# skyepurchase/MeatModeler

Hardware: AMD Instinct MI355X
Metric: descriptor-match pairs/sec + BA residuals/sec, 500×1080p frames, 1/2/4/8 GPU (higher is better)
Workload: dtype u8/int32 (match), f64 (BA); 1 GPU; 500 frames 1920x1080, 4000 ORB kpts/frame, BF Hamming 2-NN + ratio, track linking, 2-view DLT, full BA (TRF, Schur, f64 MFMA Cholesky); frames=500, height=1080, width=1920, nfeatures=4000, parallelism=pairs/points x1

## Files before the change

meatmodeler_amd/csrc/mm_common.h:

```cpp
#pragma once
#include <hip/hip_runtime.h>
#include <cstdarg>
#include <cstdio>
#include <cstring>
#include <vector>
#include "../../include/meatmodeler.h"

struct mm_prof_rec {
    const char *name;
    hipEvent_t a, b;
};

struct mm_ctx {
    int device;
    hipStream_t stream;
    char err[512];
    int prof = 0;
    char prof_only[64] = {0};
    std::vector<mm_prof_rec> recs;
    std::vector<hipEvent_t> pool;
    hipStream_t aux = nullptr;
    hipEvent_t ev_fork = nullptr, ev_join = nullptr;
    bool attr_chol_fused = false, attr_chol_bwd = false, attr_chol_batch = false;
    int cu_count = 0, fused_wgs = 0, chol_last_path = -1, debug_abandon = 0;
    bool chol_avoid_fused = false;
    bool chol_strict_budget = false;
    hipEvent_t fused_ev = nullptr;
    bool fused_ev_pending = false;
    bool fused_no_event = false;
    int link_last_variant = -1;
    void *cam_tab = nullptr;
    int cam_tab_cap = 0, cam_tab_F = 0;
    const double *cam_tab_for = nullptr;
    bool cam_tab_hold = false;
    const double *fx_cams = nullptr;
    int fx_F = 0;
    bool fx_tab_ok = false;
    void *host_board = nullptr;
    unsigned long long host_board_seq = 0;
    void *batch_dev = nullptr, *batch_host = nullptr;
    size_t batch_dev_cap = 0, batch_host_cap = 0;
    bool jvp_rows_deferred = false;
    const double *jvp_partial = nullptr;
    unsigned jvp_n_wg = 0;
    const void *chol_init_done = nullptr;
    int chol_init_sides = 0;
    int batch_last = -1;
};
// ... 54 lines not shown
    bool fused;
    int sides;
    unsigned grid_fused, grid_bwd;
};
struct mm_chol_init_args {
    int32_t *info, *flags;
    size_t nflags;
    unsigned long long *sentinel_buf;
    size_t nsent;
    unsigned long long *lpub;
    size_t nlpub;
    unsigned long long *Linv;
    size_t nblk;
};
bool mm_chol_init_plan(mm_ctx *ctx, int n, int half_bandwidth, int32_t *info, void *ws, size_t ws_bytes, mm_chol_init_args *out, int *sides, int *bwb);
void mm_chol_init_done(mm_ctx *ctx, const void *ws, int sides);
struct mm_damp_spec {
    const double *B, *C, *si;
    const double *gh2, *d11;
    double Delta, min_damping;
    double *damp_out;
    const double *reg;
};
int mm_ba_schur_solve_damped(mm_ctx *ctx, const mm_ba_problem *pb, const double *cams, const double *pts, const mm_damp_spec *dmp,
                             double *Bd, double *Cd, const double *gc, const double *gp, double *S, double *v, double *Cinv,
                             int half_bandwidth, int32_t *info, void *ws_schur, size_t ws_schur_bytes, void *ws_chol,
                             size_t ws_chol_bytes);
int mm_chol_solve_gated(mm_ctx *ctx, double *A, int n, double *b, int nrhs, int half_bandwidth, int32_t *info, void *ws,
                        size_t ws_bytes, const int32_t *slab_ready, int cams_per_slab, int n_cams, int sym_mode);

struct mm_batch_prob {
    mm_ba_problem pb;
    int64_t n, nc;
    double *x, *x_new, *g, *si, *gh, *ghs, *gn, *q1, *w, *q2, *s1, *s2;
    double *B, *Bd, *C, *Cd, *Cinv, *u1, *Jq2, *dp, *v, *S;
    double *r0, *r1, *r2, *r3, *d11, *bs, *damp, *board;
    int32_t *info;
    void *ctab_x, *ctab_new;
    double *res_partial;
    unsigned *md_counter;
    double *md_partial;
    double *jvp_partial;
    double *backsub_T;
    double *schur_partial, *schur_camtab;
    int32_t *schur_seg_done, *schur_desc;
    mm_chol_layout chol;
    int32_t half_bw, chol_sym_mirror;
    uint32_t g_vec, g_res, g_jvp, g_pblk, g_obs, g_pts, g_scale, g_damp, g_prep, g_pairs, g_chol, g_bwd, g_coef, g_zero;
    void *mailbox;
};
// ... 86 lines not shown
```

meatmodeler_amd/csrc/mm_ctx.hip:

```cpp
#include "mm_common.h"

extern "C" {

int mm_abi_version(void) { return 3; }

int mm_ctx_create(int device, void *hip_stream, mm_ctx **out) {
    if (!out) return MM_ERR_ARG;
    int n = 0;
    if (hipGetDeviceCount(&n) != hipSuccess || device < 0 || device >= n) return MM_ERR_HIP;
    mm_ctx *c = new mm_ctx();
    c->device = device;
    c->stream = (hipStream_t)hip_stream;
    c->err[0] = 0;
    if (hipSetDevice(device) != hipSuccess) {
        delete c;
        return MM_ERR_HIP;
    }
    if (hipDeviceGetAttribute(&c->cu_count, hipDeviceAttributeMultiprocessorCount, device) != hipSuccess) c->cu_count = 0;
    *out = c;
    return MM_OK;
}

void mm_ctx_destroy(mm_ctx *ctx) {
    if (!ctx) return;
// ... 68 lines not shown
const char *mm_last_error(mm_ctx *ctx) { return ctx ? ctx->err : "null context"; }

int mm_ctx_sync(mm_ctx *ctx) {
    if (!ctx) return MM_ERR_ARG;
    MM_HIP(ctx, hipStreamSynchronize(ctx->stream));
    mm_chol_release_budget(ctx);
    return MM_OK;
}

long long mm_ctx_control(mm_ctx *ctx, int what, long long value) {
    if (!ctx) return MM_ERR_ARG;
    switch (what) {
        case MM_CTL_CHOL_FORCE_ABANDON: ctx->debug_abandon = value < 0 ? 0 : (int)value; return MM_OK;
        case MM_CTL_CHOL_LAST_PATH: return ctx->chol_last_path;
        case MM_CTL_CHOL_RESERVED: return ctx->fused_wgs;
        case MM_CTL_CU_COUNT: return ctx->cu_count;
        case MM_CTL_CHOL_AVOID_FUSED: {
            const long long prev = ctx->chol_avoid_fused ? 1 : 0;
            if (value >= 0) ctx->chol_avoid_fused = value != 0;
            return prev;
        }
        case MM_CTL_LINK_LAST_VARIANT: return ctx->link_last_variant;
        case MM_CTL_BATCH_LAST: return ctx->batch_last;
        default: return mm_fail(ctx, MM_ERR_ARG, "mm_ctx_control: unknown request %d", what);
    }
}

struct mm_timer {
    hipEvent_t a, b;
};

int mm_timer_create(mm_ctx *ctx, void **timer_out) {
    if (!ctx || !timer_out) return MM_ERR_ARG;
    mm_timer *t = new mm_timer();
    MM_HIP(ctx, hipEventCreate(&t->a));
    MM_HIP(ctx, hipEventCreate(&t->b));
    *timer_out = t;
    return MM_OK;
}
int mm_timer_start(mm_ctx *ctx, void *timer) {
    if (!ctx || !timer) return MM_ERR_ARG;
    MM_HIP(ctx, hipEventRecord(((mm_timer *)timer)->a, ctx->stream));
    return MM_OK;
}
int mm_timer_stop(mm_ctx *ctx, void *timer) {
    if (!ctx || !timer) return MM_ERR_ARG;
// ... 21 lines not shown
```

meatmodeler_amd/csrc/schur.hip:

```cpp
#include "ba_eval.h"
#include "chol_init.h"

namespace {

constexpr int SR_WIN = 256;

__global__ __launch_bounds__(256) void point_inverse_kernel(int P, const double *__restrict__ Cd,
                                                            double *__restrict__ Cinv) {
    int p = blockIdx.x * 256 + threadIdx.x;
    if (p >= P) return;
    const double *c = Cd + (size_t)p * 6;
    const double a = c[0], b = c[1], d = c[2], e = c[3], f = c[4], g = c[5];
    const double m00 = e * g - f * f, m01 = d * f - b * g, m02 = b * f - d * e;
    const double det = a * m00 + b * m01 + d * m02;
    const double id = 1.0 / det;
    double *o = Cinv + (size_t)p * 6;
    o[0] = m00 * id;
    o[1] = m01 * id;
    o[2] = m02 * id;
    o[3] = (a * g - d * d) * id;
    o[4] = (b * d - a * f) * id;
    o[5] = (a * e - b * b) * id;
}

// ... 311 lines not shown
            const int sl = i / slabs.cams_per_slab;
            if (atomicAdd(slabs.done + sl, 1) == slabs.seg_count[sl] - 1)
                __hip_atomic_store(slabs.ready + sl, 1, __ATOMIC_RELEASE, __HIP_MEMORY_SCOPE_AGENT);
        }
    }
}


struct CamPQ {
    double P[9], q[3];
};
__device__ __forceinline__ double fast_rcp(double x) {
    double y = __builtin_amdgcn_rcp(x);
    double e = fma(-x, y, 1.0);
    y = fma(y, e, y);
    e = fma(-x, y, 1.0);
    return fma(y, e, y);
}

struct LeanJ {
    double Jc[2][6];
    double Jp[2][3];
};
__device__ __forceinline__ void lean_eval(const CamPQ &c, const double *__restrict__ Ks, const double *__restrict__ Jr,
                                          double X0, double X1, double X2, LeanJ &o) {
    const double u0 = fma(c.P[0], X0, fma(c.P[1], X1, fma(c.P[2], X2, c.q[0])));
    const double u1 = fma(c.P[3], X0, fma(c.P[4], X1, fma(c.P[5], X2, c.q[1])));
    const double u2 = fma(c.P[6], X0, fma(c.P[7], X1, fma(c.P[8], X2, c.q[2])));
    const double iz = fast_rcp(u2);
    const double p[2] = {u0 * iz, u1 * iz};
#pragma unroll
    for (int m = 0; m < 2; ++m) {
#pragma unroll
        for (int k = 0; k < 3; ++k) {
            o.Jp[m][k] = fma(-p[m], c.P[6 + k], c.P[3 * m + k]) * iz;
            o.Jc[m][3 + k] = fma(-p[m], Ks[6 + k], Ks[3 * m + k]) * iz;
        }
        const double g0 = X1 * o.Jp[m][2] - X2 * o.Jp[m][1];
        const double g1 = X2 * o.Jp[m][0] - X0 * o.Jp[m][2];
        const double g2 = X0 * o.Jp[m][1] - X1 * o.Jp[m][0];
#pragma unroll
        for (int k = 0; k < 3; ++k) o.Jc[m][k] = fma(g0, Jr[k], fma(g1, Jr[3 + k], g2 * Jr[6 + k]));
    }
}

constexpr int SLAB2 = 32;
struct ChunkDesc {
    int32_t i, f2, e_begin, e_end, sidx, c_first, n_ch, pad;
};
template <bool FORCE>
__device__ __forceinline__ CamPQ cam_pq_scalar(const double *__restrict__ t) {
    CamPQ v;
#pragma unroll
    for (int k = 0; k < 9; ++k) v.P[k] = FORCE ? uniform_f64(t[k]) : t[k];
#pragma unroll
    for (int k = 0; k < 3; ++k) v.q[k] = FORCE ? uniform_f64(t[9 + k]) : t[9 + k];
    return v;
}
template <bool FORCE_UNIFORM>
__device__ __forceinline__ void schur_pairs_body(const mm_ba_problem pb, const double *__restrict__ camtab,
                                                                    const ChunkDesc *__restrict__ desc,
                                                                    const double *__restrict__ pts,
                                                                    const double *__restrict__ Cinv,
                                                                    const double *__restrict__ gp,
                                                                    double *partial, const double *__restrict__ Bd,
                                                                    const double *__restrict__ gc, double *S, double *v,
// ... 43 lines not shown
#pragma unroll
    for (int q = 0; q < 42; ++q) acc[q] = 0.0;
    auto load_xc = [&](int p, double (&x)[12]) {
        if (p >= 0) {
            const double *Xp = pts + (size_t)p * 3, *ci = Cinv + (size_t)p * 6;
            x[0] = Xp[0];
            x[1] = Xp[1];
            x[2] = Xp[2];
#pragma unroll
            for (int q = 0; q < 6; ++q) x[3 + q] = ci[q];
            if (d == 0) {
                x[9] = gp[(size_t)p * 3];
                x[10] = gp[(size_t)p * 3 + 1];
                x[11] = gp[(size_t)p * 3 + 2];
            }
        }
    };
    auto pair_body = [&](int p, bool self, const double (&x)[12]) {
        const double X0 = x[0], X1 = x[1], X2 = x[2];
        const double q00 = x[3], q01 = x[4], q02 = x[5], q11 = x[6], q12 = x[7], q22 = x[8];
        LeanJ a;
        lean_eval(cp_i, Ks, Jr_i, X0, X1, X2, a);
        double Z[2][3];
#pragma unroll
        for (int m = 0; m < 2; ++m) {
            Z[m][0] = a.Jp[m][0] * q00 + a.Jp[m][1] * q01 + a.Jp[m][2] * q02;
            Z[m][1] = a.Jp[m][0] * q01 + a.Jp[m][1] * q11 + a.Jp[m][2] * q12;
            Z[m][2] = a.Jp[m][0] * q02 + a.Jp[m][1] * q12 + a.Jp[m][2] * q22;
        }
        double M[2][2], T[2][6];
        if (d == 0) {
            if (self) {
                const double g0 = x[9], g1 = x[10], g2 = x[11];
                const double z0 = Z[0][0] * g0 + Z[0][1] * g1 + Z[0][2] * g2, z1 = Z[1][0] * g0 + Z[1][1] * g1 + Z[1][2] * g2;
#pragma unroll
                for (int q = 0; q < 6; ++q) acc[36 + q] += a.Jc[0][q] * z0 + a.Jc[1][q] * z1;
            }
#pragma unroll
            for (int m = 0; m < 2; ++m)
#pragma unroll
                for (int n_ = 0; n_ < 2; ++n_) M[m][n_] = Z[m][0] * a.Jp[n_][0] + Z[m][1] * a.Jp[n_][1] + Z[m][2] * a.Jp[n_][2];
#pragma unroll
            for (int b = 0; b < 6; ++b) {
                T[0][b] = M[0][0] * a.Jc[0][b] + M[0][1] * a.Jc[1][b];
                T[1][b] = M[1][0] * a.Jc[0][b] + M[1][1] * a.Jc[1][b];
            }
        } else {
            LeanJ b2;
            lean_eval(cp_2, Ks, Jr_2, X0, X1, X2, b2);
#pragma unroll
            for (int m = 0; m < 2; ++m)
#pragma unroll
                for (int n_ = 0; n_ < 2; ++n_) M[m][n_] = Z[m][0] * b2.Jp[n_][0] + Z[m][1] * b2.Jp[n_][1] + Z[m][2] * b2.Jp[n_][2];
#pragma unroll
            for (int b = 0; b < 6; ++b) {
                T[0][b] = M[0][0] * b2.Jc[0][b] + M[0][1] * b2.Jc[1][b];
                T[1][b] = M[1][0] * b2.Jc[0][b] + M[1][1] * b2.Jc[1][b];
            }
        }
#pragma unroll
        for (int q = 0; q < 6; ++q)
#pragma unroll
            for (int b = 0; b < 6; ++b) acc[q * 6 + b] += a.Jc[0][q] * T[0][b] + a.Jc[1][q] * T[1][b];
    };
    double xc[12];
    load_xc(p_next, xc);
    int p_cur = p_next;
    bool self_cur = self_next;
    {
        const int en = e + 64;
        p_next = en < e_end ? point_of(en) : -1;
        self_next = en < e_end && self_of(en);
    }
#pragma clang loop unroll(disable)
    for (; e - lane < e_end; e += 64) {
        double xn[12];
        load_xc(p_next, xn);
        const int p_nn_e = e + 128;
        const int p_nn = p_nn_e < e_end ? point_of(p_nn_e) : -1;
        const bool self_nn = p_nn_e < e_end && self_of(p_nn_e);
        if (p_cur >= 0) pair_body(p_cur, self_cur, xc);
#pragma unroll
        for (int q = 0; q < 12; ++q) xc[q] = xn[q];
        p_cur = p_next;
        self_cur = self_next;
        p_next = p_nn;
// ... 68 lines not shown
                                                                    const double *__restrict__ gp,
                                                                    double *partial, const double *__restrict__ Bd,
                                                                    const double *__restrict__ gc, double *S, double *v,
                                                                    int32_t *seg_done, SlabSync slabs, unsigned wg_begin,
                                                                    unsigned wg_total) {
    schur_pairs_body<false>(pb, camtab, desc, pts, Cinv, gp, partial, Bd, gc, S, v, seg_done, slabs, wg_begin, wg_total, blockIdx.x);
}
__global__ __launch_bounds__(256) void zero_batch_kernel(const mm_batch_prob *__restrict__ tab, const int32_t *__restrict__ list) {
    const mm_batch_prob &bp = tab[list[blockIdx.y]];
    if (blockIdx.x >= bp.g_zero) return;
    double2 *S2 = reinterpret_cast<double2 *>(bp.S);
    const int64_t n2 = bp.nc * bp.nc / 2;
    for (int64_t i = (int64_t)blockIdx.x * 256 + threadIdx.x; i < n2; i += (int64_t)bp.g_zero * 256) S2[i] = make_double2(0.0, 0.0);
}
__global__ __launch_bounds__(64 * SP_WAVES, 2) void schur_pairs_batch_kernel(const mm_batch_prob *__restrict__ tab, const int32_t *__restrict__ list) {
    const mm_batch_prob &bp = tab[list[blockIdx.y]];
    if (blockIdx.x >= bp.g_pairs) return;
    SlabSync none = {};
    schur_pairs_body<true>(bp.pb, bp.schur_camtab, (const ChunkDesc *)bp.schur_desc, bp.x + bp.nc, bp.Cinv, bp.g + bp.nc, bp.schur_partial, bp.Bd,
                     bp.g, bp.S, bp.v, bp.schur_seg_done, none, 0u, bp.g_pairs, blockIdx.x);
}




__global__ void slab_flag_kernel(int32_t *flags, int s) {
    __hip_atomic_store(flags + s, 1, __ATOMIC_RELEASE, __HIP_MEMORY_SCOPE_AGENT);
}

__global__ void schur_diag_fill_kernel(mm_ba_problem pb, const double *__restrict__ Bd, const double *__restrict__ gc,
                                       double *__restrict__ S, double *__restrict__ v) {
    const int i = blockIdx.x;
    if (pb.cam_ptr[i + 1] != pb.cam_ptr[i]) return;
    const size_t n = (size_t)pb.F * 6;
    if (threadIdx.x < 36) S[((size_t)i * 6 + threadIdx.x / 6) * n + (size_t)i * 6 + threadIdx.x % 6] = Bd[(size_t)i * 36 + threadIdx.x];
    if (threadIdx.x < 6) v[(size_t)i * 6 + threadIdx.x] = gc[(size_t)i * 6 + threadIdx.x];
}

struct PrepExtra {
    mm_damp_spec dmp;
    int zero_bwb;
    int chol_init;
    mm_chol_init_args init;
};
__device__ __forceinline__ void schur_prepare_body(mm_ba_problem pb, const double *__restrict__ cams,
                                                            double *__restrict__ Bd, const double *__restrict__ Cd,
// ... 167 lines not shown
    if (pb->O == 0) return MM_OK;
    MM_LAUNCH(ctx, "pairs_count_kernel", pairs_count_kernel, dim3((unsigned)((pb->O + 255) / 256)), dim3(256), 0, *pb, cnt,
              span_out);
    return MM_OK;
}

extern "C" int mm_ba_pairs_emit(mm_ctx *ctx, const mm_ba_problem *pb, const int64_t *offsets, int span, int32_t *key,
                                int32_t *pair_o, int32_t *pair_o2) {
    if (!ctx) return MM_ERR_ARG;
    if (!pb || !offsets || !key || !pair_o || !pair_o2 || span < 0) return mm_fail(ctx, MM_ERR_ARG, "mm_ba_pairs_emit: bad argument");
    if (pb->O == 0) return MM_OK;
    if ((int64_t)pb->F * (span + 1) > 0x7fffffffLL) return mm_fail(ctx, MM_ERR_ARG, "mm_ba_pairs_emit: F * (span + 1) overflows the key");
    MM_LAUNCH(ctx, "pairs_emit_kernel", pairs_emit_kernel, dim3((unsigned)((pb->O + 255) / 256)), dim3(256), 0, *pb, offsets,
              span, key, pair_o, pair_o2);
    return MM_OK;
}

extern "C" size_t mm_ba_schur_workspace_bytes(const mm_ba_problem *pb) {
    if (!pb || pb->n_chunks <= 0) return 0;
    return mm_align_up((size_t)pb->n_chunks * 42 * sizeof(double), 256)  +
           mm_align_up((size_t)pb->n_seg * sizeof(int32_t), 256)  +
           mm_align_up(2 * MAX_SLABS * sizeof(int32_t), 256)  +
           mm_align_up((size_t)pb->F * CAMTAB2 * sizeof(double), 256)  +
           mm_align_up((size_t)pb->n_chunks * 32, 256) ;
}

namespace {
bool schur_pairs_lean() {
    static const bool lean = [] {
        const char *e = getenv("MM_SCHUR_PAIRS");
        return !(e && e[0] == 'r');
    }();
    return lean;
}
#define MM_LAUNCH_PAIRS(ctx, grid, pbv, camtab_, desc_, ...)                                                             \
    do {                                                                                                                 \
        if (schur_pairs_lean())                                                                                          \
            MM_LAUNCH(ctx, "schur_pairs_kernel", schur_pairs_kernel<2>, grid, dim3(64 * SP_WAVES), 0, pbv, camtab_,      \
                      (const ChunkDesc *)(desc_), __VA_ARGS__);                                                          \
        else                                                                                                             \
            MM_LAUNCH(ctx, "schur_pairs_ref_kernel", schur_pairs_ref_kernel, grid, dim3(64 * SP_WAVES), 0, pbv, camtab_, \
                      __VA_ARGS__);                                                                                      \
    } while (0)
struct SchurWs {
    double *partial, *camtab;
    int32_t *seg_done, *slab_ready, *slab_done, *desc;
};
SchurWs carve_schur_ws(const mm_ba_problem *pb, void *ws) {
    SchurWs w;
    char *p = (char *)ws;
    w.partial = (double *)p;
    p += mm_align_up((size_t)pb->n_chunks * 42 * sizeof(double), 256);
    w.seg_done = (int32_t *)p;
    p += mm_align_up((size_t)pb->n_seg * sizeof(int32_t), 256);
    w.slab_ready = (int32_t *)p;
    w.slab_done = w.slab_ready + MAX_SLABS;
    p += mm_align_up(2 * MAX_SLABS * sizeof(int32_t), 256);
    w.camtab = (double *)p;
    p += mm_align_up((size_t)pb->F * CAMTAB2 * sizeof(double), 256);
    w.desc = (int32_t *)p;
    return w;
}
}

extern "C" int mm_ba_schur(mm_ctx *ctx, const mm_ba_problem *pb, const double *cams, const double *pts,
                           const double *Bd, const double *Cd, const double *gc, const double *gp, double *S, double *v,
                           double *Cinv, void *ws, size_t ws_bytes) {
    if (!ctx) return MM_ERR_ARG;
    if (!pb || pb->F < 0 || pb->P < 0 || pb->O < 0 || !pb->K) return mm_fail(ctx, MM_ERR_ARG, "mm_ba_schur: bad problem");
    if (!cams || !pts || !Bd || !Cd || !gc || !gp || !S || !v || !Cinv || !pb->pt_ptr || !pb->cam_ptr ||
        (pb->O > 0 && (!pb->pt_obs || !pb->cam_obs || !pb->fi || !pb->pi || !pb->obs)))
        return mm_fail(ctx, MM_ERR_ARG, "mm_ba_schur: null pointer");
    if (pb->F == 0) return MM_OK;
    if (pb->n_seg > 0 && pb->n_chunks > 0 && pb->seg_ids && pb->seg_chunk_ptr && pb->chunk_seg && pb->chunk_begin &&
        pb->chunk_end && pb->pair_o && pb->pair_o2) {
        if (!ws || ws_bytes < mm_ba_schur_workspace_bytes(pb)) return mm_fail(ctx, MM_ERR_WORKSPACE, "mm_ba_schur: workspace too small");
        MM_HIP(ctx, hipMemsetAsync(S, 0, (size_t)pb->F * 6 * pb->F * 6 * sizeof(double), ctx->stream));
        const int64_t wgs = (pb->n_chunks + SP_WAVES - 1) / SP_WAVES;
        const SchurWs w = carve_schur_ws(pb, ws);
        SlabSync none = {};
        const int prep = (pb->P + 255) / 256 > pb->F ? (pb->P + 255) / 256 : pb->F;
        MM_LAUNCH(ctx, "schur_prepare_kernel", schur_prepare_kernel, dim3(prep), dim3(256), 0, *pb, cams, const_cast<double *>(Bd), Cd, gc,
                  Cinv, S, v, w.camtab, w.seg_done, schur_pairs_lean(), schur_pairs_lean() ? w.desc : (int32_t *)nullptr);
// ... 57 lines not shown
    const unsigned wg_total = (unsigned)((pb->n_chunks + SP_WAVES - 1) / SP_WAVES);
    const unsigned wg_first = wg_total / 2;
    if (wg_first > 0)
        MM_LAUNCH_PAIRS(ctx, dim3(wg_first), *pb, (const double *)w.camtab, w.desc, pts, (const double *)Cinv, gp, w.partial, Bd, gc, S, v,
                        w.seg_done, slabs, 0u, wg_total);
    MM_HIP(ctx, hipEventRecord(ctx->ev_fork, ctx->stream));
    MM_HIP(ctx, hipStreamWaitEvent(ctx->aux, ctx->ev_fork, 0));
    {
        mm_stream_swap sw(ctx, ctx->aux);
        int rc = mm_chol_solve_gated(ctx, S, n, v, 1, half_bandwidth, info, ws_chol, ws_chol_bytes, w.slab_ready, cams_per_slab, pb->F, 2);
        if (rc) {
            (void)hipEventRecord(ctx->ev_join, ctx->aux);
            (void)hipStreamWaitEvent(sw.saved, ctx->ev_join, 0);
            return rc;
        }
        MM_HIP(ctx, hipEventRecord(ctx->ev_join, ctx->aux));
    }
    MM_LAUNCH_PAIRS(ctx, dim3(wg_total - wg_first), *pb, (const double *)w.camtab, w.desc, pts, (const double *)Cinv, gp, w.partial, Bd, gc, S, v,
                    w.seg_done, slabs, wg_first, wg_total);
    MM_HIP(ctx, hipStreamWaitEvent(ctx->stream, ctx->ev_join, 0));
    return MM_OK;
}

int mm_ba_schur_solve_damped(mm_ctx *ctx, const mm_ba_problem *pb, const double *cams, const double *pts, const mm_damp_spec *dmp,
                             double *Bd, double *Cd, const double *gc, const double *gp, double *S, double *v, double *Cinv,
                             int half_bandwidth, int32_t *info, void *ws_schur, size_t ws_schur_bytes, void *ws_chol,
                             size_t ws_chol_bytes) {
    if (!ctx) return MM_ERR_ARG;
    if (!pb || !dmp || !info || !cams || !pts || !Bd || !gc || !gp || !S || !v || !Cinv || !dmp->B || !dmp->C || !dmp->si ||
        (!dmp->gh2 && !dmp->reg) || (dmp->gh2 && (!dmp->d11 || !dmp->damp_out)))
        return mm_fail(ctx, MM_ERR_ARG, "mm_ba_schur_solve_damped: bad argument");
    const int n = pb->F * 6;
    static const bool off = [] { const char *e = getenv("MM_SCHUR_FOLD"); return e && atoi(e) == 0; }();
    mm_chol_init_args ia = {};
    int sides = 0, bwb = 0;
    const bool pairs_ok = pb->n_seg > 0 && pb->n_chunks > 0 && pb->seg_ids && pb->seg_chunk_ptr && pb->chunk_seg && pb->chunk_begin &&
                          pb->chunk_end && pb->pair_o && pb->pair_o2 && pb->P > 0 && schur_pairs_lean();
    const bool fold = !off && pairs_ok && ws_schur && ws_schur_bytes >= mm_ba_schur_workspace_bytes(pb) &&
                      mm_chol_init_plan(ctx, n, half_bandwidth, info, ws_chol, ws_chol_bytes, &ia, &sides, &bwb);
    if (!fold) {
        if (!Cd) return mm_fail(ctx, MM_ERR_ARG, "mm_ba_schur_solve_damped: the separate calls need Cd");
        int rc = dmp->gh2 ? mm_ba_damp_damping(ctx, pb->F, pb->P, dmp->B, dmp->C, dmp->si, dmp->gh2, dmp->d11, dmp->Delta, dmp->min_damping,
                                                dmp->damp_out, Bd, Cd)
                          : mm_ba_damp(ctx, pb->F, pb->P, dmp->B, dmp->C, dmp->si, dmp->reg, Bd, Cd);
        if (rc) return rc;
        return mm_ba_schur_solve(ctx, pb, cams, pts, Bd, Cd, gc, gp, S, v, Cinv, half_bandwidth, info, ws_schur, ws_schur_bytes, ws_chol,
                                 ws_chol_bytes, 0, 0, nullptr, nullptr);
    }
    const SchurWs w = carve_schur_ws(pb, ws_schur);
    PrepExtra ex = {};
    ex.dmp = *dmp;
    ex.zero_bwb = bwb;
    ex.chol_init = 1;
    ex.init = ia;
    const int prep = (pb->P + 255) / 256 > pb->F ? (pb->P + 255) / 256 : pb->F;
    MM_LAUNCH(ctx, "schur_prepare_kernel", schur_prepare_damped_kernel, dim3(prep), dim3(256), 0, *pb, cams, Bd, gc, Cinv, S, v, w.camtab,
              w.seg_done, w.desc, ex);
    const int64_t wgs = (pb->n_chunks + SP_WAVES - 1) / SP_WAVES;
    SlabSync none = {};
    MM_LAUNCH_PAIRS(ctx, dim3((unsigned)wgs), *pb, (const double *)w.camtab, w.desc, pts, (const double *)Cinv, gp, w.partial,
                    (const double *)Bd, gc, S, v, w.seg_done, none, 0u, (unsigned)wgs);
    mm_chol_init_done(ctx, ws_chol, sides);
    const int rc = mm_chol_solve_sym(ctx, S, n, v, half_bandwidth, 1, info, ws_chol, ws_chol_bytes);
    mm_chol_init_done(ctx, nullptr, 0);
    return rc;
}

int mm_batch_schur_setup(mm_ctx *ctx, mm_batch_prob *bp, void *ws_schur, size_t ws_schur_bytes) {
    const mm_ba_problem *pb = &bp->pb;
    if (!(pb->n_seg > 0 && pb->n_chunks > 0 && pb->seg_ids && pb->seg_chunk_ptr && pb->chunk_seg && pb->chunk_begin && pb->chunk_end &&
          pb->pair_o && pb->pair_o2 && pb->pair_p) || pb->P <= 0)
        return mm_fail(ctx, MM_ERR_ARG, "mm_ba_trf_batched: a problem without a co-observation pair list");
    if (!ws_schur || ws_schur_bytes < mm_ba_schur_workspace_bytes(pb)) return mm_fail(ctx, MM_ERR_WORKSPACE, "mm_ba_trf_batched: Schur workspace");
    const SchurWs w = carve_schur_ws(pb, ws_schur);
    bp->schur_partial = w.partial;
    bp->schur_camtab = w.camtab;
    bp->schur_seg_done = w.seg_done;
    bp->schur_desc = w.desc;
    bp->g_prep = (uint32_t)((pb->P + 255) / 256 > pb->F ? (pb->P + 255) / 256 : pb->F);
    bp->g_pairs = (uint32_t)((pb->n_chunks + SP_WAVES - 1) / SP_WAVES);
    const int64_t n2 = bp->nc * bp->nc / 2;
    const int64_t gz = (n2 + 2047) / 2048;
    bp->g_zero = (uint32_t)(gz < 1 ? 1 : (gz > 1024 ? 1024 : gz));
    return MM_OK;
// ... 10 lines not shown
```

meatmodeler_amd/csrc/trf.hip:

```cpp
#include "mm_common.h"
#include "trf_decide.h"
#include <chrono>
#include <vector>
#include <algorithm>
#include <initializer_list>
#include <utility>
#include <cmath>
#include <cstdlib>

namespace {

__global__ __launch_bounds__(256) void vec_mul_kernel(const double *__restrict__ a, const double *__restrict__ b,
                                                      double *__restrict__ out, int64_t n) {
    const int64_t i = (int64_t)blockIdx.x * 256 + threadIdx.x;
    if (i < n) out[i] = a[i] * b[i];
}

struct HostBoard {
    double v[16];
    unsigned long long seq;
    unsigned long long pad[7];
};

__global__ __launch_bounds__(64) void board_publish_kernel(const double *__restrict__ dev, int count, HostBoard *hb,
// ... 273 lines not shown
        TRF_CALL(ar(t.ex, (int64_t)F * 42));
        MM_HIP(ctx, hipMemcpyAsync(t.B, t.ex, (size_t)F * 36 * sizeof(double), hipMemcpyDeviceToDevice, st));
        MM_HIP(ctx, hipMemcpyAsync(t.g, t.ex + (size_t)F * 36, (size_t)nc * sizeof(double), hipMemcpyDeviceToDevice, st));
        return MM_OK;
    };
    if (!ctx->host_board) {
        MM_HIP(ctx, hipHostMalloc(&ctx->host_board, sizeof(HostBoard), hipHostMallocDefault));
        memset(ctx->host_board, 0, sizeof(HostBoard));
        ctx->host_board_seq = 0;
    }
    HostBoard *hb = (HostBoard *)ctx->host_board;
    auto take_board = [&](unsigned long long seq, int count) -> int {
        TRF_CALL(wait_seq(ctx, &hb->seq, seq, "mm_ba_trf: the trial-step scalars"));
        for (int i = 0; i < count; ++i) host[i] = ((volatile double *)hb->v)[i];
        mm_chol_release_budget(ctx);
        return MM_OK;
    };
    auto read_board = [&](const double *dev, int count) -> int {
        const unsigned long long seq = ++ctx->host_board_seq;
        hipLaunchKernelGGL(board_publish_kernel, dim3(1), dim3(64), 0, st, dev, count, hb, seq);
        MM_LAUNCH_CHECK(ctx, "board_publish_kernel");
        return take_board(seq, count);
    };
    TRF_CALL(mm_ba_residual(ctx, pb, x, pts_of(x), nullptr, t.cost2, t.ws_res, t.ws_res_b));
    if (dist) {
        const double av = ctx->chol_avoid_fused ? 1.0 : 0.0;
        MM_HIP(ctx, hipMemcpyAsync(t.board + 15, &av, sizeof(double), hipMemcpyHostToDevice, st));
        MM_HIP(ctx, hipStreamSynchronize(st));
        TRF_CALL(exchange({{t.cost2, 3}, {t.board + 15, 3}}));
        TRF_CALL(read_board(t.board + 15, 1));
        if (host[0] > 0) ctx->chol_avoid_fused = true;
    }
    TRF_CALL(read_board(t.cost2, 1));
    const double cost0 = 0.5 * host[0];
    rep->cost0 = cost0;
    if (!std::isfinite(cost0)) {
        rep->status = -2;
        return mm_fail(ctx, MM_ERR_NUMERIC, "mm_ba_trf: residuals are not finite in the initial point");
    }
    const int half_bw = dist ? dist->half_bandwidth : 6 * pb->cam_span + 5;
    TRF_CALL(normal_eq(x));
    TRF_CALL(mm_ba_scale_update(ctx, F, P, t.B, t.C, t.si, 1));
    {
        hipLaunchKernelGGL(vec_mul_kernel, dim3((unsigned)((n + 255) / 256)), dim3(256), 0, st, (const double *)x, (const double *)t.si, t.w, n);
        const double *pa[1] = {t.w}, *pbv[1] = {t.w};
        TRF_CALL(mm_multi_dot(ctx, 1, pa, pbv, n, nc, t.rowsx, t.ws_md, t.ws_md_b));
        TRF_CALL(exchange({{t.rowsx, 0}}));
        TRF_CALL(read_board(t.rowsx, 3));
    }
    TrfDecide d(cost0, host[2], n, *prm, log, log_cap);
    Outcome next = d.begin();
    static const bool timing = getenv("MM_TRF_TIMING") && atoi(getenv("MM_TRF_TIMING")) > 0;
    const auto t_loop = std::chrono::steady_clock::now();
    auto t_iter = t_loop;
    if (timing) fprintf(stderr, "mm_ba_trf timing: prologue %.1f us\n", std::chrono::duration<double, std::micro>(t_loop - t_enter).count());
    for (;;) {
        if (timing && d.iteration > 0) {
            const auto now = std::chrono::steady_clock::now();
            fprintf(stderr, "mm_ba_trf timing: iteration %d %.1f us (nfev %d)\n", d.iteration - 1,
                    std::chrono::duration<double, std::micro>(now - t_iter).count(), d.nfev);
            t_iter = now;
// ... 34 lines not shown
                mm_cam_table_invalidate(ctx);
            }
            if (!dist) {
                const unsigned long long seq = ++ctx->host_board_seq;
                TRF_CALL(mm_ba_residual_publish(ctx, pb, x_new, pts_of(x_new), t.ws_res, t.ws_res_b, t.board, 14, 16,
                                                ctx->host_board, seq));
                return take_board(seq, 16);
            }
            TRF_CALL(mm_ba_residual(ctx, pb, x_new, pts_of(x_new), nullptr, t.board + 14, t.ws_res, t.ws_res_b));
            TRF_CALL(exchange({{t.board + 14, 3}, {t.board + 15, 4}}));
            return read_board(t.board, 16);
        };
        bool damping_known = false;
        Outcome solve;
        do {
            if (!dist) {
                mm_damp_spec dmp = {t.B, t.C, t.si, nullptr, nullptr, d.Delta, d.min_damping, t.damp, reg_eff};
                if (!damping_known) {
                    dmp.gh2 = t.r0 + 2;
                    dmp.d11 = t.d11 + 2;
                    damping_known = true;
                }
                TRF_CALL(mm_ba_schur_solve_damped(ctx, pb, x, pts_of(x), &dmp, t.Bd, t.Cd, t.g, pts_of(t.g), t.S, t.v, t.Cinv,
                                                  half_bw, t.info, t.ws_schur, t.ws_schur_b, t.ws_chol, t.ws_chol_b));
            } else {
                if (!damping_known) {
                    TRF_CALL(mm_ba_damp_damping(ctx, F, P, t.B, t.C, t.si, t.r0 + 2, t.d11 + 2, d.Delta, d.min_damping, t.damp, t.Bd, t.Cd));
                    damping_known = true;
                } else {
                    TRF_CALL(mm_ba_damp(ctx, F, P, t.B, t.C, t.si, reg_eff, t.Bd, t.Cd));
                }
                TRF_CALL(mm_ba_schur(ctx, pb, x, pts_of(x), t.Bd, t.Cd, t.g, pts_of(t.g), t.S, t.v, t.Cinv, t.ws_schur,
                                     t.ws_schur_b));
                const double dup = (double)(dist->world - 1);
                if (dist->band_exchange) {
                    const int hb = (int)(half_bw < nc - 1 ? half_bw : nc - 1);
                    const int64_t cnt = nc * (hb + 1);
                    hipLaunchKernelGGL(band_pack_kernel, dim3((unsigned)((cnt + 255) / 256)), dim3(256), 0, st, (const double *)t.S, nc, hb, t.ex);
                    MM_HIP(ctx, hipMemcpyAsync(t.ex + cnt, t.v, (size_t)nc * sizeof(double), hipMemcpyDeviceToDevice, st));
                    TRF_CALL(ar(t.ex, cnt + nc));
                    hipLaunchKernelGGL(band_unpack_kernel, dim3((unsigned)((cnt + 255) / 256)), dim3(256), 0, st, t.S, nc, hb,
                                       (const double *)t.ex, (const double *)t.Bd, dup);
                    MM_HIP(ctx, hipMemcpyAsync(t.v, t.ex + cnt, (size_t)nc * sizeof(double), hipMemcpyDeviceToDevice, st));
                } else {
                    MM_HIP(ctx, hipMemcpyAsync(t.S + nc * nc, t.v, (size_t)nc * sizeof(double), hipMemcpyDeviceToDevice, st));
                    TRF_CALL(ar(t.S, nc * nc + nc));
                    MM_HIP(ctx, hipMemcpyAsync(t.v, t.S + nc * nc, (size_t)nc * sizeof(double), hipMemcpyDeviceToDevice, st));
// ... 332 lines not shown
```

Baseline: 9253 billion descriptor pairs/s (match stage).

## Split short Schur pair chunks into a dedicated small-chunk kernel

Once per TRF solve, the chunk list is partitioned on device into regular chunks and short single-chunk off-diagonal segments (at most 16 pairs). The regular ones go to the existing pairs kernel. The short ones go to a new kernel that packs four chunks per 64-lane wave and writes the 6x6 S blocks directly, aiming to cut the wasted lanes and reduction overhead of the full pairs kernel on tiny chunks. This adds a count/place pass, a host readback of the counts, extra workspace, and two pair-kernel launches per Schur build. The stage being changed is bundle adjustment, while the reported metric is descriptor matching.

```diff
diff --git a/meatmodeler_amd/csrc/mm_common.h b/meatmodeler_amd/csrc/mm_common.h
--- a/meatmodeler_amd/csrc/mm_common.h
+++ b/meatmodeler_amd/csrc/mm_common.h
@@ -24,6 +24,7 @@
     bool attr_chol_fused = false, attr_chol_bwd = false, attr_chol_batch = false;
     int cu_count = 0, fused_wgs = 0, chol_last_path = -1, debug_abandon = 0;
     bool chol_avoid_fused = false;
+    int schur_small = 1;
     bool chol_strict_budget = false;
     hipEvent_t fused_ev = nullptr;
     bool fused_ev_pending = false;
@@ -124,10 +125,19 @@
     double *damp_out;
     const double *reg;
 };
+struct mm_schur_split {
+    int64_t n_rest, n_small;
+    int mode;
+};
+int mm_ba_schur_split(mm_ctx *ctx, const mm_ba_problem *pb, void *ws_schur, size_t ws_schur_bytes, const double **counts);
 int mm_ba_schur_solve_damped(mm_ctx *ctx, const mm_ba_problem *pb, const double *cams, const double *pts, const mm_damp_spec *dmp,
                              double *Bd, double *Cd, const double *gc, const double *gp, double *S, double *v, double *Cinv,
                              int half_bandwidth, int32_t *info, void *ws_schur, size_t ws_schur_bytes, void *ws_chol,
-                             size_t ws_chol_bytes);
+                             size_t ws_chol_bytes, const mm_schur_split *split);
+#define MM_CTL_SCHUR_SMALL 8
+extern "C" int mm_ba_schur_split_build(mm_ctx *ctx, const mm_ba_problem *pb, const double *cams, const double *pts, const double *Bd,
+                                       const double *Cd, const double *gc, const double *gp, double *S, double *v, double *Cinv,
+                                       void *ws, size_t ws_bytes);
 int mm_chol_solve_gated(mm_ctx *ctx, double *A, int n, double *b, int nrhs, int half_bandwidth, int32_t *info, void *ws,
                         size_t ws_bytes, const int32_t *slab_ready, int cams_per_slab, int n_cams, int sym_mode);
 
diff --git a/meatmodeler_amd/csrc/mm_ctx.hip b/meatmodeler_amd/csrc/mm_ctx.hip
--- a/meatmodeler_amd/csrc/mm_ctx.hip
+++ b/meatmodeler_amd/csrc/mm_ctx.hip
@@ -114,6 +114,12 @@
         }
         case MM_CTL_LINK_LAST_VARIANT: return ctx->link_last_variant;
         case MM_CTL_BATCH_LAST: return ctx->batch_last;
+        case MM_CTL_SCHUR_SMALL: {
+            const long long prev = ctx->schur_small;
+            if (value > 2) return mm_fail(ctx, MM_ERR_ARG, "mm_ctx_control: MM_CTL_SCHUR_SMALL takes 0, 1 or 2");
+            if (value >= 0) ctx->schur_small = (int)value;
+            return prev;
+        }
         default: return mm_fail(ctx, MM_ERR_ARG, "mm_ctx_control: unknown request %d", what);
     }
 }
diff --git a/meatmodeler_amd/csrc/schur.hip b/meatmodeler_amd/csrc/schur.hip
--- a/meatmodeler_amd/csrc/schur.hip
+++ b/meatmodeler_amd/csrc/schur.hip
@@ -357,7 +357,8 @@
     double Jc[2][6];
     double Jp[2][3];
 };
-__device__ __forceinline__ void lean_eval(const CamPQ &c, const double *__restrict__ Ks, const double *__restrict__ Jr,
+template <class CAM>
+__device__ __forceinline__ void lean_eval(const CAM &c, const double *__restrict__ Ks, const double *__restrict__ Jr,
                                           double X0, double X1, double X2, LeanJ &o) {
     const double u0 = fma(c.P[0], X0, fma(c.P[1], X1, fma(c.P[2], X2, c.q[0])));
     const double u1 = fma(c.P[3], X0, fma(c.P[4], X1, fma(c.P[5], X2, c.q[1])));
@@ -377,6 +378,31 @@
 #pragma unroll
         for (int k = 0; k < 3; ++k) o.Jc[m][k] = fma(g0, Jr[k], fma(g1, Jr[3 + k], g2 * Jr[6 + k]));
     }
+}
+__device__ __forceinline__ void pair_Z(const LeanJ &a, double q00, double q01, double q02, double q11, double q12, double q22,
+                                       double (&Z)[2][3]) {
+#pragma unroll
+    for (int m = 0; m < 2; ++m) {
+        Z[m][0] = a.Jp[m][0] * q00 + a.Jp[m][1] * q01 + a.Jp[m][2] * q02;
+        Z[m][1] = a.Jp[m][0] * q01 + a.Jp[m][1] * q11 + a.Jp[m][2] * q12;
+        Z[m][2] = a.Jp[m][0] * q02 + a.Jp[m][1] * q12 + a.Jp[m][2] * q22;
+    }
+}
+__device__ __forceinline__ void pair_M(const double (&Z)[2][3], const LeanJ &b2, double (&M)[2][2]) {
+#pragma unroll
+    for (int m = 0; m < 2; ++m)
+#pragma unroll
+        for (int n_ = 0; n_ < 2; ++n_) M[m][n_] = Z[m][0] * b2.Jp[n_][0] + Z[m][1] * b2.Jp[n_][1] + Z[m][2] * b2.Jp[n_][2];
+}
+__device__ __forceinline__ void pair_T(const double (&M)[2][2], const LeanJ &b2, double (&T)[2][6]) {
+#pragma unroll
+    for (int b = 0; b < 6; ++b) {
+        T[0][b] = M[0][0] * b2.Jc[0][b] + M[0][1] * b2.Jc[1][b];
+        T[1][b] = M[1][0] * b2.Jc[0][b] + M[1][1] * b2.Jc[1][b];
+    }
+}
+__device__ __forceinline__ void pair_add(double &sum, const LeanJ &a, const double (&T)[2][6], int q, int b) {
+    sum += a.Jc[0][q] * T[0][b] + a.Jc[1][q] * T[1][b];
 }
 
 constexpr int SLAB2 = 32;
@@ -466,12 +492,7 @@
         LeanJ a;
         lean_eval(cp_i, Ks, Jr_i, X0, X1, X2, a);
         double Z[2][3];
-#pragma unroll
-        for (int m = 0; m < 2; ++m) {
-            Z[m][0] = a.Jp[m][0] * q00 + a.Jp[m][1] * q01 + a.Jp[m][2] * q02;
-            Z[m][1] = a.Jp[m][0] * q01 + a.Jp[m][1] * q11 + a.Jp[m][2] * q12;
-            Z[m][2] = a.Jp[m][0] * q02 + a.Jp[m][1] * q12 + a.Jp[m][2] * q22;
-        }
+        pair_Z(a, q00, q01, q02, q11, q12, q22, Z);
         double M[2][2], T[2][6];
         if (d == 0) {
             if (self) {
@@ -505,7 +526,7 @@
 #pragma unroll
         for (int q = 0; q < 6; ++q)
 #pragma unroll
-            for (int b = 0; b < 6; ++b) acc[q * 6 + b] += a.Jc[0][q] * T[0][b] + a.Jc[1][q] * T[1][b];
+            for (int b = 0; b < 6; ++b) pair_add(acc[q * 6 + b], a, T, q, b);
     };
     double xc[12];
     load_xc(p_next, xc);
@@ -620,6 +641,166 @@
 }
 
 
+
+constexpr int SMALL_MAX = 16;
+constexpr int SMALL_CAM_LD = 56;
+struct CamLds {
+    const double *P, *q;
+};
+__device__ __forceinline__ bool chunk_is_short(const mm_ba_problem &pb, int64_t k) {
+    const int sidx = pb.chunk_seg[k];
+    return pb.seg_chunk_ptr[sidx + 1] - pb.seg_chunk_ptr[sidx] == 1 && pb.chunk_end[k] - pb.chunk_begin[k] <= SMALL_MAX &&
+           pb.seg_ids[sidx] % (pb.cam_span + 1) != 0;
+}
+__global__ __launch_bounds__(64, 4) void schur_pairs_small_kernel(mm_ba_problem pb, const double *__restrict__ camtab,
+                                                                  const ChunkDesc *__restrict__ desc, int n_small,
+                                                                  const double *__restrict__ pts, const double *__restrict__ Cinv,
+                                                                  double *__restrict__ S) {
+    __shared__ double Ks[9];
+    __shared__ double cam[4][SMALL_CAM_LD];
+    __shared__ int32_t who[4][2];
+    __shared__ double red[12 * RED_LD];
+    const int lane = threadIdx.x, g = lane >> 4, j = lane & 15;
+    if (lane < 9) Ks[lane] = pb.K[lane];
+    const int64_t k = (int64_t)blockIdx.x * 4 + g;
+    const bool live = k < n_small;
+    int i = -1, f2 = -1, e = 0;
+    bool has = false;
+    if (live) {
+        const ChunkDesc cd = desc[k];
+        i = cd.i;
+        f2 = cd.f2;
+        e = cd.e_begin + j;
+        has = e < cd.e_end;
+    }
+    double X0 = 0.0, X1 = 0.0, X2 = 0.0, q00 = 0.0, q01 = 0.0, q02 = 0.0, q11 = 0.0, q12 = 0.0, q22 = 0.0;
+    if (live) {
+#pragma unroll
+        for (int t = 0; t < 3; ++t) {
+            const int idx = j + 16 * t;
+            cam[g][idx] = camtab[(size_t)(idx < CAMTAB2 ? i : f2) * CAMTAB2 + (idx < CAMTAB2 ? idx : idx - CAMTAB2)];
+        }
+    }
+    if (j == 0) {
+        who[g][0] = i;
+        who[g][1] = f2;
+    }
+    if (has) {
+        const int p = pb.pair_p ? pb.pair_p[e] : pb.pi[pb.pair_o[e]];
+        const double *Xp = pts + (size_t)p * 3, *ci = Cinv + (size_t)p * 6;
+        X0 = Xp[0], X1 = Xp[1], X2 = Xp[2];
+        q00 = ci[0], q01 = ci[1], q02 = ci[2], q11 = ci[3], q12 = ci[4], q22 = ci[5];
+    }
+    __syncthreads();
+    LeanJ a;
+    double T[2][6];
+    if (has) {
+        const double *ca = cam[g], *cb = cam[g] + CAMTAB2;
+        const CamLds cp_i = {ca, ca + 9}, cp_2 = {cb, cb + 9};
+        lean_eval(cp_i, Ks, ca + 12, X0, X1, X2, a);
+        double Z[2][3], M[2][2];
+        pair_Z(a, q00, q01, q02, q11, q12, q22, Z);
+        LeanJ b2;
+        lean_eval(cp_2, Ks, cb + 12, X0, X1, X2, b2);
+        pair_M(Z, b2, M);
+        pair_T(M, b2, T);
+    }
+    const size_t n = (size_t)pb.F * 6;
+    const int rg = lane / 12, rw = lane % 12;
+#pragma unroll
+    for (int r = 0; r < 3; ++r) {
+#pragma unroll
+        for (int w = 0; w < 12; ++w) {
+            double val = 0.0;
+            if (has) pair_add(val, a, T, 2 * r + w / 6, w % 6);
+            red[w * RED_LD + lane] = val;
+        }
+        wave_lds_barrier();
+        if (lane < 48) {
+            const double *row = red + rw * RED_LD + 16 * rg;
+            double s0 = 0.0, s1 = 0.0, s2 = 0.0, s3 = 0.0;
+#pragma unroll
+            for (int jj = 0; jj < 16; jj += 4) {
+                s0 += row[jj];
+                s1 += row[jj + 1];
+                s2 += row[jj + 2];
+                s3 += row[jj + 3];
+            }
+            s0 += 0.0;
+            s1 += 0.0;
+            s2 += 0.0;
+            s3 += 0.0;
+            const double val = -((s0 + s1) + (s2 + s3));
+            const int ri = who[rg][0], rf = who[rg][1];
+            if (ri >= 0) {
+                const int q = 12 * r + rw;
+                S[((size_t)ri * 6 + q / 6) * n + (size_t)rf * 6 + q % 6] = val;
+                S[((size_t)rf * 6 + q % 6) * n + (size_t)ri * 6 + q / 6] = val;
+            }
+        }
+        wave_lds_barrier();
+    }
+}
+
+constexpr int SPLIT_TILE = 1024;
+__global__ __launch_bounds__(SPLIT_TILE) void schur_split_count_kernel(mm_ba_problem pb, int32_t *__restrict__ tile_short) {
+    const int64_t k = (int64_t)blockIdx.x * SPLIT_TILE + threadIdx.x;
+    const int n = __syncthreads_count(k < pb.n_chunks && chunk_is_short(pb, k));
+    if (threadIdx.x == 0) tile_short[blockIdx.x] = n;
+}
+__global__ __launch_bounds__(SPLIT_TILE) void schur_split_place_kernel(mm_ba_problem pb, const int32_t *__restrict__ tile_short,
+                                                                       int32_t *__restrict__ split, double *__restrict__ counts) {
+    __shared__ int32_t wave_sum[SPLIT_TILE / 64], tot[2][SPLIT_TILE / 64];
+    const int tid = threadIdx.x, lane = tid & 63, wv = tid >> 6;
+    int before = 0, all = 0;
+    for (int t = tid; t < (int)gridDim.x; t += SPLIT_TILE) {
+        const int c = tile_short[t];
+        all += c;
+        if (t < (int)blockIdx.x) before += c;
+    }
+    for (int off = 32; off > 0; off >>= 1) {
+        before += __shfl_down(before, off, 64);
+        all += __shfl_down(all, off, 64);
+    }
+    if (lane == 0) {
+        tot[0][wv] = before;
+        tot[1][wv] = all;
+    }
+    __syncthreads();
+    before = 0;
+    all = 0;
+    for (int w = 0; w < SPLIT_TILE / 64; ++w) {
+        before += tot[0][w];
+        all += tot[1][w];
+    }
+    const int64_t n_rest = pb.n_chunks - all;
+    if (blockIdx.x == 0 && tid == 0) {
+        counts[0] = (double)n_rest;
+        counts[1] = (double)all;
+    }
+    const int64_t k = (int64_t)blockIdx.x * SPLIT_TILE + tid;
+    const bool in = k < pb.n_chunks;
+    const bool sh = in && chunk_is_short(pb, k);
+    const unsigned long long m = __ballot(sh);
+    const int in_wave = __popcll(m & ((1ull << lane) - 1));
+    if (lane == 0) wave_sum[wv] = __popcll(m);
+    __syncthreads();
+    int sb = before + in_wave;
+    for (int w = 0; w < wv; ++w) sb += wave_sum[w];
+    if (!in) return;
+    const int sidx = pb.chunk_seg[k], seg = pb.seg_ids[sidx];
+    const int ci = seg / (pb.cam_span + 1), cdd = seg % (pb.cam_span + 1);
+    const int c_first = pb.seg_chunk_ptr[sidx];
+    int32_t *o = split + 8 * (sh ? n_rest + sb : k - sb);
+    o[0] = ci;
+    o[1] = ci - cdd;
+    o[2] = pb.chunk_begin[k];
+    o[3] = pb.chunk_end[k];
+    o[4] = sidx;
+    o[5] = c_first - sb;
+    o[6] = pb.seg_chunk_ptr[sidx + 1] - c_first;
+    o[7] = 0;
+}
 
 
 __global__ void slab_flag_kernel(int32_t *flags, int s) {
@@ -833,7 +1014,10 @@
            mm_align_up((size_t)pb->n_seg * sizeof(int32_t), 256)  +
            mm_align_up(2 * MAX_SLABS * sizeof(int32_t), 256)  +
            mm_align_up((size_t)pb->F * CAMTAB2 * sizeof(double), 256)  +
-           mm_align_up((size_t)pb->n_chunks * 32, 256) ;
+           mm_align_up((size_t)pb->n_chunks * 32, 256)  +
+           mm_align_up((size_t)pb->n_chunks * 32, 256)  +
+           mm_align_up((size_t)((pb->n_chunks + SPLIT_TILE - 1) / SPLIT_TILE) * sizeof(int32_t), 256)  +
+           256 ;
 }
 
 namespace {
@@ -856,6 +1040,8 @@
 struct SchurWs {
     double *partial, *camtab;
     int32_t *seg_done, *slab_ready, *slab_done, *desc;
+    int32_t *split, *tile_short;
+    double *split_counts;
 };
 SchurWs carve_schur_ws(const mm_ba_problem *pb, void *ws) {
     SchurWs w;
@@ -870,6 +1056,12 @@
     w.camtab = (double *)p;
     p += mm_align_up((size_t)pb->F * CAMTAB2 * sizeof(double), 256);
     w.desc = (int32_t *)p;
+    p += mm_align_up((size_t)pb->n_chunks * 32, 256);
+    w.split = (int32_t *)p;
+    p += mm_align_up((size_t)pb->n_chunks * 32, 256);
+    w.tile_short = (int32_t *)p;
+    p += mm_align_up((size_t)((pb->n_chunks + SPLIT_TILE - 1) / SPLIT_TILE) * sizeof(int32_t), 256);
+    w.split_counts = (double *)p;
     return w;
 }
 }
@@ -973,10 +1165,80 @@
     return MM_OK;
 }
 
+namespace {
+bool schur_pairs_ok(const mm_ba_problem *pb) {
+    return pb->n_seg > 0 && pb->n_chunks > 0 && pb->seg_ids && pb->seg_chunk_ptr && pb->chunk_seg && pb->chunk_begin && pb->chunk_end &&
+           pb->pair_o && pb->pair_o2;
+}
+int launch_pairs_split(mm_ctx *ctx, const mm_ba_problem *pb, const SchurWs &w, const mm_schur_split *sp, const double *pts,
+                       const double *Cinv, const double *gp, const double *Bd, const double *gc, double *S, double *v) {
+    SlabSync none = {};
+    mm_ba_problem rest = *pb;
+    rest.n_chunks = sp->n_rest;
+    if (sp->n_rest > 0)
+        MM_LAUNCH(ctx, "schur_pairs_kernel", schur_pairs_kernel<2>, dim3((unsigned)sp->n_rest), dim3(64 * SP_WAVES), 0, rest,
+                  (const double *)w.camtab, (const ChunkDesc *)w.split, pts, Cinv, gp, w.partial, Bd, gc, S, v, w.seg_done, none, 0u,
+                  (unsigned)sp->n_rest);
+    if (sp->n_small <= 0) return MM_OK;
+    const ChunkDesc *small = (const ChunkDesc *)w.split + sp->n_rest;
+    if (sp->mode == 2) {
+        mm_ba_problem sh = *pb;
+        sh.n_chunks = sp->n_small;
+        MM_LAUNCH(ctx, "schur_pairs_kernel_short", schur_pairs_kernel<2>, dim3((unsigned)sp->n_small), dim3(64 * SP_WAVES), 0, sh,
+                  (const double *)w.camtab, small, pts, Cinv, gp, w.partial, Bd, gc, S, v, w.seg_done, none, 0u, (unsigned)sp->n_small);
+        return MM_OK;
+    }
+    MM_LAUNCH(ctx, "schur_pairs_small_kernel", schur_pairs_small_kernel, dim3((unsigned)((sp->n_small + 3) / 4)), dim3(64), 0, *pb,
+              (const double *)w.camtab, small, (int)sp->n_small, pts, Cinv, S);
+    return MM_OK;
+}
+}
+
+int mm_ba_schur_split(mm_ctx *ctx, const mm_ba_problem *pb, void *ws_schur, size_t ws_schur_bytes, const double **counts) {
+    if (!ctx) return MM_ERR_ARG;
+    if (!pb || !counts) return mm_fail(ctx, MM_ERR_ARG, "mm_ba_schur_split: bad argument");
+    *counts = nullptr;
+    if (ctx->schur_small == 0 || !schur_pairs_ok(pb) || pb->P <= 0 || !schur_pairs_lean() || !ws_schur ||
+        ws_schur_bytes < mm_ba_schur_workspace_bytes(pb))
+        return MM_OK;
+    const SchurWs w = carve_schur_ws(pb, ws_schur);
+    const unsigned tiles = (unsigned)((pb->n_chunks + SPLIT_TILE - 1) / SPLIT_TILE);
+    MM_LAUNCH(ctx, "schur_split_kernel", schur_split_count_kernel, dim3(tiles), dim3(SPLIT_TILE), 0, *pb, w.tile_short);
+    MM_LAUNCH(ctx, "schur_split_kernel", schur_split_place_kernel, dim3(tiles), dim3(SPLIT_TILE), 0, *pb, (const int32_t *)w.tile_short,
+              w.split, w.split_counts);
+    *counts = w.split_counts;
+    return MM_OK;
+}
+
+extern "C" int mm_ba_schur_split_build(mm_ctx *ctx, const mm_ba_problem *pb, const double *cams, const double *pts, const double *Bd,
+                                       const double *Cd, const double *gc, const double *gp, double *S, double *v, double *Cinv,
+                                       void *ws, size_t ws_bytes) {
+    if (!ctx) return MM_ERR_ARG;
+    if (!pb || !cams || !pts || !Bd || !Cd || !gc || !gp || !S || !v || !Cinv || pb->F <= 0 || !pb->K || !schur_pairs_ok(pb) ||
+        !schur_pairs_lean())
+        return mm_fail(ctx, MM_ERR_ARG, "mm_ba_schur_split_build: bad argument (needs the pair list)");
+    const double *counts = nullptr;
+    int rc = mm_ba_schur_split(ctx, pb, ws, ws_bytes, &counts);
+    if (rc) return rc;
+    if (!counts) return mm_ba_schur(ctx, pb, cams, pts, Bd, Cd, gc, gp, S, v, Cinv, ws, ws_bytes);
+    double h[2];
+    MM_HIP(ctx, hipMemcpyAsync(h, counts, sizeof(h), hipMemcpyDeviceToHost, ctx->stream));
+    MM_HIP(ctx, hipStreamSynchronize(ctx->stream));
+    const mm_schur_split sp = {(int64_t)h[0], (int64_t)h[1], ctx->schur_small};
+    if (sp.n_rest < 0 || sp.n_small < 0 || sp.n_rest + sp.n_small != pb->n_chunks)
+        return mm_fail(ctx, MM_ERR_NUMERIC, "mm_ba_schur_split_build: the lists do not add up");
+    MM_HIP(ctx, hipMemsetAsync(S, 0, (size_t)pb->F * 6 * pb->F * 6 * sizeof(double), ctx->stream));
+    const SchurWs w = carve_schur_ws(pb, ws);
+    const int prep = (pb->P + 255) / 256 > pb->F ? (pb->P + 255) / 256 : pb->F;
+    MM_LAUNCH(ctx, "schur_prepare_kernel", schur_prepare_kernel, dim3(prep), dim3(256), 0, *pb, cams, const_cast<double *>(Bd), Cd, gc, Cinv,
+              S, v, w.camtab, w.seg_done, true, (int32_t *)nullptr);
+    return launch_pairs_split(ctx, pb, w, &sp, pts, Cinv, gp, Bd, gc, S, v);
+}
+
 int mm_ba_schur_solve_damped(mm_ctx *ctx, const mm_ba_problem *pb, const double *cams, const double *pts, const mm_damp_spec *dmp,
                              double *Bd, double *Cd, const double *gc, const double *gp, double *S, double *v, double *Cinv,
                              int half_bandwidth, int32_t *info, void *ws_schur, size_t ws_schur_bytes, void *ws_chol,
-                             size_t ws_chol_bytes) {
+                             size_t ws_chol_bytes, const mm_schur_split *split) {
     if (!ctx) return MM_ERR_ARG;
     if (!pb || !dmp || !info || !cams || !pts || !Bd || !gc || !gp || !S || !v || !Cinv || !dmp->B || !dmp->C || !dmp->si ||
         (!dmp->gh2 && !dmp->reg) || (dmp->gh2 && (!dmp->d11 || !dmp->damp_out)))
@@ -1005,12 +1267,18 @@
     ex.chol_init = 1;
     ex.init = ia;
     const int prep = (pb->P + 255) / 256 > pb->F ? (pb->P + 255) / 256 : pb->F;
+    const bool use_split = split && split->mode != 0 && split->n_rest + split->n_small == pb->n_chunks;
     MM_LAUNCH(ctx, "schur_prepare_kernel", schur_prepare_damped_kernel, dim3(prep), dim3(256), 0, *pb, cams, Bd, gc, Cinv, S, v, w.camtab,
-              w.seg_done, w.desc, ex);
-    const int64_t wgs = (pb->n_chunks + SP_WAVES - 1) / SP_WAVES;
-    SlabSync none = {};
-    MM_LAUNCH_PAIRS(ctx, dim3((unsigned)wgs), *pb, (const double *)w.camtab, w.desc, pts, (const double *)Cinv, gp, w.partial,
-                    (const double *)Bd, gc, S, v, w.seg_done, none, 0u, (unsigned)wgs);
+              w.seg_done, use_split ? (int32_t *)nullptr : w.desc , ex);
+    if (use_split) {
+        const int rc = launch_pairs_split(ctx, pb, w, split, pts, Cinv, gp, Bd, gc, S, v);
+        if (rc) return rc;
+    } else {
+        const int64_t wgs = (pb->n_chunks + SP_WAVES - 1) / SP_WAVES;
+        SlabSync none = {};
+        MM_LAUNCH_PAIRS(ctx, dim3((unsigned)wgs), *pb, (const double *)w.camtab, w.desc, pts, (const double *)Cinv, gp, w.partial,
+                        (const double *)Bd, gc, S, v, w.seg_done, none, 0u, (unsigned)wgs);
+    }
     mm_chol_init_done(ctx, ws_chol, sides);
     const int rc = mm_chol_solve_sym(ctx, S, n, v, half_bandwidth, 1, info, ws_chol, ws_chol_bytes);
     mm_chol_init_done(ctx, nullptr, 0);
diff --git a/meatmodeler_amd/csrc/trf.hip b/meatmodeler_amd/csrc/trf.hip
--- a/meatmodeler_amd/csrc/trf.hip
+++ b/meatmodeler_amd/csrc/trf.hip
@@ -319,6 +319,9 @@
         MM_LAUNCH_CHECK(ctx, "board_publish_kernel");
         return take_board(seq, count);
     };
+    const double *split_counts = nullptr;
+    mm_schur_split split = {0, 0, 0};
+    if (!dist) TRF_CALL(mm_ba_schur_split(ctx, pb, t.ws_schur, t.ws_schur_b, &split_counts));
     TRF_CALL(mm_ba_residual(ctx, pb, x, pts_of(x), nullptr, t.cost2, t.ws_res, t.ws_res_b));
     if (dist) {
         const double av = ctx->chol_avoid_fused ? 1.0 : 0.0;
@@ -334,6 +337,12 @@
     if (!std::isfinite(cost0)) {
         rep->status = -2;
         return mm_fail(ctx, MM_ERR_NUMERIC, "mm_ba_trf: residuals are not finite in the initial point");
+    }
+    if (split_counts) {
+        TRF_CALL(read_board(split_counts, 2));
+        split.n_rest = (int64_t)host[0];
+        split.n_small = (int64_t)host[1];
+        split.mode = ctx->schur_small;
     }
     const int half_bw = dist ? dist->half_bandwidth : 6 * pb->cam_span + 5;
     TRF_CALL(normal_eq(x));
@@ -414,7 +423,8 @@
                     damping_known = true;
                 }
                 TRF_CALL(mm_ba_schur_solve_damped(ctx, pb, x, pts_of(x), &dmp, t.Bd, t.Cd, t.g, pts_of(t.g), t.S, t.v, t.Cinv,
-                                                  half_bw, t.info, t.ws_schur, t.ws_schur_b, t.ws_chol, t.ws_chol_b));
+                                                  half_bw, t.info, t.ws_schur, t.ws_schur_b, t.ws_chol, t.ws_chol_b,
+                                                  split_counts ? &split : nullptr));
             } else {
                 if (!damping_known) {
                     TRF_CALL(mm_ba_damp_damping(ctx, F, P, t.B, t.C, t.si, t.r0 + 2, t.d11 + 2, d.Delta, d.min_damping, t.damp, t.Bd, t.Cd));
```

After: 9129 billion descriptor pairs/s (match stage). 0.987x the previous value.
